# Scalsol/mega.pytorch

Hardware: AMD Instinct MI355X
Metric: frames/sec MEGA R-101 inference, 1000x600 VID clip (higher is better)
Workload: dtype bf16

## Files before the change

### include/mega_hip.h

```cpp
#ifndef MEGA_HIP_H
#define MEGA_HIP_H

#include <stddef.h>

#ifdef __cplusplus
extern "C" {
#endif

#define MEGA_F32 0
#define MEGA_BF16 1
#define MEGA_F16 2

#define MEGA_OK 0
#define MEGA_ERR_ARG 1
#define MEGA_ERR_LAUNCH 2
#define MEGA_ERR_WS 3
#define MEGA_ERR_LIMIT 4

int mega_conv2d_nhwc(const void* in, const void* w, const float* scale, const float* bias, const void* residual,
                     void* out, int N, int H, int W, int Cin, int Cout, int R, int S, int stride, int pad, int dil,
                     int relu, int ldo, int ldr, int in_dtype, int out_dtype, void* stream);
int mega_conv2d_nhwc_tile(int M, int Cout, int K);
int mega_conv2d_nhwc_plan(int M, int Cout, int K, int in_dtype);
int mega_conv2d_nhwc_plan_ex(int N, int H, int W, int Cin, int Cout, int R, int S, int stride, int pad, int dil, int ldo,
                             int has_residual, int in_dtype, int out_dtype);

size_t mega_conv2d_nhwc_workspace_bytes(int M, int Cout, int K);
int mega_conv2d_nhwc_ws(const void* in, const void* w, const float* scale, const float* bias, const void* residual,
                        void* out, int N, int H, int W, int Cin, int Cout, int R, int S, int stride, int pad, int dil,
                        int relu, int ldo, int ldr, int in_dtype, int out_dtype, void* ws, size_t ws_bytes, void* stream);

int mega_conv2d_nhwc_rs(const void* in, const void* w, const float* scale, const float* bias, const void* residual, void* out,
                        int N, int H, int W, int Cin, int Cout, int relu, int ldo, int ldr, int res_H, int res_W, int res_stride,
                        int dtype, void* stream);

int mega_stem_conv_bn_relu(const float* in, const float* w_tap64, const float* scale, const float* bias, void* out,
                           int N, int H, int W, int out_dtype, void* stream);
int mega_stem_conv_bn_relu_bf16(const float* in, const void* w_n176_bf16, const float* scale, const float* bias,
                                void* out, int N, int H, int W, void* stream);
int mega_stem_conv_bn_relu_bf16_u8(const void* frames_u8, const void* w_n176_bf16, const float* scale, const float* bias,
                                   void* out, int N, int H, int W, float mean0, float mean1, float mean2, int to_bgr,
                                   void* stream);

int mega_stem_pool_dt(const void* in, int u8, const void* w_n176, const float* scale, const float* bias, void* out, int N,
                      int H, int W, float mean0, float mean1, float mean2, int to_bgr, int dtype, void* stream);
void mega_stem_pool_tile(int* rows, int* cols);

int mega_maxpool3x3s2_nhwc(const void* in, void* out, int N, int H, int W, int C, int dtype, void* stream);

int mega_avgpool2x2_ceil_nhwc(const void* in, void* out, int N, int H, int W, int C, int dtype, void* stream);

int mega_roi_align_fwd(const void* feat, const float* rois, void* out, int K, int C, int H, int W,
                       float spatial_scale, int pooled_h, int pooled_w, int sampling_ratio, int in_nhwc,
                       int out_nhwc, int dtype, int out_dtype, void* stream);

size_t mega_nms_full_workspace_bytes(int n);
int mega_nms(const float* dets, const float* scores, int n, float thr, int strict_gt, long long* keep_out,
             int* keep_cnt, void* ws, size_t ws_bytes, void* stream);

size_t mega_nms_workspace_bytes(int P, int nmax);
int mega_nms_sorted(const float* boxes, const int* counts, const unsigned char* valid, const int* order, int P,
                    int nmax, float thr, int strict_gt, int max_keep, int* keep_pos, int* keep_cnt,
                    unsigned char* flags, void* ws, size_t ws_bytes, void* stream);

size_t mega_rpn_select_workspace_bytes(int B, int pre_nms_top_n);
int mega_rpn_select_idx(const float* rpn_out, const float* cell_anchors, int B, int Hf, int Wf, int A, int ldc,
                        int anchor_stride, int pre_nms_top_n, int post_nms_top_n, float nms_thresh, int strict_gt,
                        float min_size, float im_w, float im_h, float* proposals, float* prop_scores, int* prop_cnt,
                        int* prop_index, void* ws, size_t ws_bytes, void* stream);

size_t mega_postprocess_workspace_bytes(int R, int NC);
int mega_postprocess(const float* logits, const float* deltas, const float* props, const int* nprop, int R, int NC,
                     float wx, float wy, float ww, float wh, float im_w, float im_h, float score_thresh,
                     float nms_thresh, int strict_gt, int max_det, float* out_boxes, float* out_scores,
                     long long* out_labels, int* out_cnt, float* probs_out, void* ws, size_t ws_bytes,
                     void* stream);

size_t mega_postprocess_batched_workspace_bytes(int B, int R, int NC);
int mega_postprocess_batched(const float* logits, const float* deltas, const float* props, const int* nprop, int B,
                             int R, int NC, float wx, float wy, float ww, float wh, float im_w, float im_h,
                             float score_thresh, float nms_thresh, int strict_gt, int max_det, float* out_boxes,
                             float* out_scores, long long* out_labels, int* out_cnt, float* probs_out, void* ws,
                             size_t ws_bytes, void* stream);

int mega_postprocess_candidates_batched(const float* logits, const float* deltas, const float* props, const int* nprop,
                                        int B, int R, int NC, float wx, float wy, float ww, float wh, float im_w,
                                        float im_h, float score_thresh, float* cboxes, float* cscores, void* stream);

size_t mega_bbox_aug_merge_workspace_bytes(int F, int K, int R, int NC);
int mega_bbox_aug_merge(const float* cboxes, const float* cscores, int F, int K, int R, int NC, const int* view_w,
                        const int* view_h, const int* view_flip, float score_thresh, float nms_thresh, int strict_gt,
                        int max_det, float* out_boxes, float* out_scores, long long* out_labels, int* out_cnt, void* ws,
                        size_t ws_bytes, void* stream);

size_t mega_soft_merge_workspace_bytes(int F, int K, int R, int NC);
int mega_soft_merge(const float* cboxes, const float* cscores, int F, int K, int R, int NC, const int* view_w,
                    const int* view_h, const int* view_flip, float score_thresh, float nms_thresh, int strict_gt,
                    int soft_method, float sigma, int vote, float vote_thresh, int vote_scoring, int max_det,
                    float* out_boxes, float* out_scores, long long* out_labels, int* out_cnt, void* ws, size_t ws_bytes,
                    void* stream);

int mega_position_logits(const float* rois_q, const float* rois_k, const float* wg_t, const float* bg,
                         const float* dim_mat, float* out, int Nq, int Nk, int ldp, int precise, void* stream);

int mega_relation_attention(const void* q, int ldq, const void* k, int ldk, const void* vt, int ldv,
                            const float* pos, int ldp, const void* resid, int ldr, const float* bias_v, void* out,
                            int ldo, int Nq, int Nk, int groups, float scale, int dtype, void* ws, size_t ws_bytes,
                            void* stream);
int mega_relation_attention_splits(int Nq, int Nk, int groups);
size_t mega_relation_attention_workspace_bytes(int Nq, int Nk, int groups);

int mega_preprocess_frames(const unsigned char* in, float* out, int N, int H, int W, float mean0, float mean1,
                           float mean2, int to_bgr, void* stream);

int mega_resize_bilinear_u8(const unsigned char* in, unsigned char* out, unsigned char* tmp, int N, int Hi, int Wi,
                            int Ho, int Wo, const int* bounds_h, const int* coef_h, int ksize_h, const int* bounds_v,
                            const int* coef_v, int ksize_v, void* stream);
int mega_resize_bilinear_u8_flip(const unsigned char* in, unsigned char* out, unsigned char* tmp, int N, int Hi, int Wi,
                                 int Ho, int Wo, const int* bounds_h, const int* coef_h, int ksize_h,
                                 const int* bounds_v, const int* coef_v, int ksize_v, int hflip, void* stream);

int mega_fgfa_warp_aggregate(const void* feats, const float* flow, void* out, float* weights_out, int T, int H,
                             int W, int Cf, int Ce, int key, int dtype, void* stream);
int mega_fgfa_warp_aggregate_ring(const void* feats, const float* flow, void* out, float* weights_out, int T, int H,
                                  int W, int Cf, int Ce, const int* order, int dtype, void* stream);

int mega_fgfa_pair_taps(const float* ring, long long ring_stride, const float* cur, long long cur_stride, const int* order,
                        void* out, int T, int H, int W, int dtype, void* stream);

int mega_dff_warp_scale(const void* feats, const float* flow, const void* scale, void* out, int H, int W, int C,
                        int dtype, void* stream);

int mega_copy_segments(const void* segs, int n, void* stream);

int mega_bottleneck64_fwd_dt(const void* x, const void* w1, const float* s1, const float* b1, const void* w2, const float* s2,
                             const float* b2, const void* w3, const float* s3, const float* b3, void* out, int N, int H, int W,
                             int dtype, void* stream);

int mega_bottleneck64_even_fwd_dt(const void* x, const void* w1, const float* s1, const float* b1, const void* w2, const float* s2,
                                  const float* b2, const void* w3, const float* s3, const float* b3, void* out, int N, int H, int W,
                                  int dtype, void* stream);

int mega_bottleneck64_ds_fwd_dt(const void* x, const void* w1, const float* s1, const float* b1, const void* w2, const float* s2,
                                const float* b2, const void* w3, const float* s3, const float* b3, const void* wd, const float* sd,
                                const float* bd, void* out, int N, int H, int W, int dtype, void* stream);

int mega_split_f32_to_bf16x3(const float* src, void* dst_bf16, int rows, int K, void* stream);


int mega_split_f32_to_planes_dt(const float* src, void* dst, int rows, int K, int dtype, void* stream);

int mega_roi_align_fwd_planes_dt(const float* feat, const float* rois, void* out_planes, int K, int C, int H, int W,
                                 float spatial_scale, int pooled_h, int pooled_w, int sampling_ratio, int dtype, void* stream);

int mega_conv2d_nhwc_sp_dt(const void* in, int ldi, int kwrap, const void* w, const float* scale, const float* bias,
                           const void* residual, int ldr, void* out, int ldo, int out_mode, int N, int H, int W, int Cin,
                           int Cout, int R, int S, int stride, int pad, int dil, int relu, int dtype, void* ws, size_t ws_bytes,
                           void* stream);


int mega_copy_cast_segments_dt(const void* segs, int n, int dtype, void* stream);

int mega_cast_f32_to_half(const float* src, void* dst, size_t n, int dtype, void* stream);

const char* mega_last_error_string(void);

typedef struct {
  const void* q; const void* k; const void* vt; const float* pos; const void* pos_tiled; const void* resid;
  const float* bias_v; void* out; void* ws; size_t ws_bytes;
  int ldq, ldk, ldv, ldp, ldr, ldo, Nq, Nk;
  int io_f32;
  int nk1;
  const void* k2;
  const void* vt2;
  int ldv2;
  int reserved;
} mega_attn_desc;
int mega_relation_attention_batched(const void* descs , int n, int groups,
                                    float scale, int dtype, void* stream);

typedef struct { const float* rois_q; const float* rois_k; void* out_bf16; int Nq, Nk; } mega_pos_desc;

int mega_position_logits_tiled_dt(const float* rois_q, const float* rois_k, const float* wg_t, const float* bg,
                                  const float* dim_mat, void* out16, int Nq, int Nk, int dtype, void* stream);
int mega_position_logits_tiled_batched_dt(const void* descs , int n, const float* wg_t,
                                          const float* bg, const float* dim_mat, int dtype, void* stream);
int mega_relation_attention_tiled_pos_dt(const void* q, int ldq, const void* k, int ldk, const void* vt, int ldv,
// ... 75 lines not shown
```

### mega/pytorch_amd/_lib.py

```python
import ctypes
import os

HERE = os.path.dirname(os.path.abspath(__file__))
LIB_PATH = os.path.join(HERE, "libmega_hip.so")

c_int, c_float, c_void_p, c_size_t = ctypes.c_int, ctypes.c_float, ctypes.c_void_p, ctypes.c_size_t
c_longlong = ctypes.c_longlong

_ERR = {1: "bad argument", 2: "kernel launch failure", 3: "workspace too small", 4: "kernel loop bound exceeded"}

SIGNATURES = {
    "mega_conv2d_nhwc": (c_int, [c_void_p] * 6 + [c_int] * 15 + [c_void_p]),
    "mega_conv2d_nhwc_ws": (c_int, [c_void_p] * 6 + [c_int] * 15 + [c_void_p, c_size_t, c_void_p]),
    "mega_conv2d_nhwc_workspace_bytes": (c_size_t, [c_int] * 3),
    "mega_conv2d_nhwc_rs": (c_int, [c_void_p] * 6 + [c_int] * 12 + [c_void_p]),
    "mega_stem_conv_bn_relu": (c_int, [c_void_p] * 5 + [c_int] * 4 + [c_void_p]),
    "mega_stem_conv_bn_relu_bf16": (c_int, [c_void_p] * 5 + [c_int] * 3 + [c_void_p]),
    "mega_stem_conv_bn_relu_bf16_u8": (c_int, [c_void_p] * 5 + [c_int] * 3 + [c_float] * 3 + [c_int, c_void_p]),
    "mega_stem_pool_dt": (c_int, [c_void_p, c_int] + [c_void_p] * 4 + [c_int] * 3 + [c_float] * 3 + [c_int, c_int, c_void_p]),
    "mega_stem_pool_tile": (None, [c_void_p, c_void_p]),
    "mega_maxpool3x3s2_nhwc": (c_int, [c_void_p] * 2 + [c_int] * 5 + [c_void_p]),
    "mega_avgpool2x2_ceil_nhwc": (c_int, [c_void_p] * 2 + [c_int] * 5 + [c_void_p]),
    "mega_roi_align_fwd": (c_int, [c_void_p] * 3 + [c_int] * 4 + [c_float] + [c_int] * 7 + [c_void_p]),
    "mega_nms_full_workspace_bytes": (c_size_t, [c_int]),
    "mega_nms": (c_int, [c_void_p, c_void_p, c_int, c_float, c_int, c_void_p, c_void_p, c_void_p, c_size_t, c_void_p]),
    "mega_nms_workspace_bytes": (c_size_t, [c_int, c_int]),
    "mega_nms_sorted": (c_int, [c_void_p] * 4 + [c_int, c_int, c_float, c_int, c_int] + [c_void_p] * 4 +
                        [c_size_t, c_void_p]),
    "mega_rpn_select_workspace_bytes": (c_size_t, [c_int, c_int]),
    "mega_rpn_select_idx": (c_int, [c_void_p, c_void_p] + [c_int] * 8 + [c_float, c_int, c_float, c_float, c_float] +
                            [c_void_p] * 5 + [c_size_t, c_void_p]),
    "mega_postprocess_workspace_bytes": (c_size_t, [c_int, c_int]),
    "mega_postprocess": (c_int, [c_void_p] * 4 + [c_int, c_int] + [c_float] * 8 + [c_int, c_int] + [c_void_p] * 6 +
                         [c_size_t, c_void_p]),
    "mega_postprocess_batched_workspace_bytes": (c_size_t, [c_int, c_int, c_int]),
    "mega_postprocess_batched": (c_int, [c_void_p] * 4 + [c_int, c_int, c_int] + [c_float] * 8 + [c_int, c_int] +
                                 [c_void_p] * 6 + [c_size_t, c_void_p]),
    "mega_postprocess_candidates_batched": (c_int, [c_void_p] * 4 + [c_int] * 3 + [c_float] * 7 + [c_void_p] * 3),
    "mega_bbox_aug_merge_workspace_bytes": (c_size_t, [c_int] * 4),
    "mega_bbox_aug_merge": (c_int, [c_void_p, c_void_p] + [c_int] * 4 + [c_void_p] * 3 + [c_float, c_float, c_int, c_int] +
                            [c_void_p] * 5 + [c_size_t, c_void_p]),
    "mega_soft_merge_workspace_bytes": (c_size_t, [c_int] * 4),
    "mega_soft_merge": (c_int, [c_void_p, c_void_p] + [c_int] * 4 + [c_void_p] * 3 +
                        [c_float, c_float, c_int, c_int, c_float, c_int, c_float, c_int, c_int] + [c_void_p] * 5 +
                        [c_size_t, c_void_p]),
    "mega_position_logits": (c_int, [c_void_p] * 6 + [c_int] * 4 + [c_void_p]),
    "mega_relation_attention_splits": (c_int, [c_int, c_int, c_int]),
    "mega_relation_attention_workspace_bytes": (c_size_t, [c_int, c_int, c_int]),
    "mega_relation_attention": (c_int, [c_void_p, c_int, c_void_p, c_int, c_void_p, c_int, c_void_p, c_int,
                                        c_void_p, c_int, c_void_p, c_void_p, c_int, c_int, c_int, c_int, c_float,
                                        c_int, c_void_p, c_size_t, c_void_p]),
    "mega_relation_attention_batched": (c_int, [c_void_p, c_int, c_int, c_float, c_int, c_void_p]),
    "mega_position_logits_tiled_dt": (c_int, [c_void_p] * 6 + [c_int] * 3 + [c_void_p]),
    "mega_position_logits_tiled_batched_dt": (c_int, [c_void_p, c_int, c_void_p, c_void_p, c_void_p, c_int, c_void_p]),
    "mega_relation_attention_tiled_pos_dt": (c_int, [c_void_p, c_int, c_void_p, c_int, c_void_p, c_int, c_void_p,
                                                     c_void_p, c_int, c_void_p, c_void_p, c_int, c_int, c_int, c_int,
                                                     c_float, c_int, c_void_p, c_size_t, c_void_p]),
    "mega_conv2d_nhwc_tile": (c_int, [c_int] * 3),
    "mega_conv2d_nhwc_plan": (c_int, [c_int] * 4),
    "mega_conv2d_nhwc_plan_ex": (c_int, [c_int] * 14),
    "mega_preprocess_frames": (c_int, [c_void_p, c_void_p] + [c_int] * 3 + [c_float] * 3 + [c_int, c_void_p]),
    "mega_dff_warp_scale": (c_int, [c_void_p] * 4 + [c_int] * 4 + [c_void_p]),
    "mega_fgfa_pair_taps": (c_int, [c_void_p, c_longlong, c_void_p, c_longlong, c_void_p, c_void_p] + [c_int] * 4 + [c_void_p]),
    "mega_resize_bilinear_u8": (c_int, [c_void_p] * 3 + [c_int] * 5 + [c_void_p, c_void_p, c_int, c_void_p, c_void_p,
                                                                      c_int, c_void_p]),
    "mega_resize_bilinear_u8_flip": (c_int, [c_void_p] * 3 + [c_int] * 5 + [c_void_p, c_void_p, c_int, c_void_p,
                                                                           c_void_p, c_int, c_int, c_void_p]),
    "mega_fgfa_warp_aggregate": (c_int, [c_void_p] * 4 + [c_int] * 7 + [c_void_p]),
    "mega_fgfa_warp_aggregate_ring": (c_int, [c_void_p] * 4 + [c_int] * 5 + [c_void_p, c_int, c_void_p]),
    "mega_copy_segments": (c_int, [c_void_p, c_int, c_void_p]),
    "mega_bottleneck64_fwd_dt": (c_int, [c_void_p] * 11 + [c_int] * 4 + [c_void_p]),
    "mega_bottleneck64_even_fwd_dt": (c_int, [c_void_p] * 11 + [c_int] * 4 + [c_void_p]),
    "mega_bottleneck64_ds_fwd_dt": (c_int, [c_void_p] * 14 + [c_int] * 4 + [c_void_p]),
    "mega_cast_f32_to_half": (c_int, [c_void_p, c_void_p, c_size_t, c_int, c_void_p]),
    "mega_copy_cast_segments_dt": (c_int, [c_void_p, c_int, c_int, c_void_p]),
    "mega_split_f32_to_bf16x3": (c_int, [c_void_p, c_void_p, c_int, c_int, c_void_p]),
    "mega_split_f32_to_planes_dt": (c_int, [c_void_p, c_void_p, c_int, c_int, c_int, c_void_p]),
    "mega_roi_align_fwd_planes_dt": (c_int, [c_void_p] * 3 + [c_int] * 4 + [c_float] + [c_int] * 4 + [c_void_p]),
    "mega_conv2d_nhwc_sp_dt": (c_int, [c_void_p, c_int, c_int, c_void_p, c_void_p, c_void_p, c_void_p, c_int, c_void_p, c_int,
                                       c_int] + [c_int] * 12 + [c_void_p, c_size_t, c_void_p]),
    "mega_conv2d_nhwc_ks_workspace_bytes": (c_size_t, [c_int] * 5),
    "mega_conv2d_nhwc_ks": (c_int, [c_void_p] * 6 + [c_int] * 16 + [c_void_p, c_size_t, c_void_p]),
    "mega_conv2d_nhwc_subpixel": (c_int, [c_void_p] * 4 + [c_int] * 13 + [c_void_p, c_size_t, c_void_p]),
    "mega_flow_level_assemble": (c_int, [c_void_p] * 5 + [c_int] * 10 + [c_void_p]),
    "mega_flow_pred_finish": (c_int, [c_void_p, c_int, c_void_p, c_float, c_void_p] + [c_int] * 4 + [c_void_p]),
    "mega_flow_conv1_combine": (c_int, [c_void_p, c_void_p, c_void_p, c_int, c_void_p, c_int, c_longlong, c_int, c_int, c_void_p]),
    "mega_fgfa_warp_aggregate_ring_pos": (c_int, [c_void_p] * 4 + [c_int] * 5 + [c_void_p, c_int, c_int, c_void_p]),
    "mega_fgfa_warp_aggregate_ring_pos_batched": (c_int, [c_void_p] * 4 + [c_int] * 5 + [c_void_p, c_int, c_int, c_int, c_void_p]),
    "mega_vid_eval_match": (c_int, [c_void_p] * 10 + [c_int] * 3 + [c_longlong, c_int] + [c_void_p] * 4),
    "mega_vid_eval_workspace_bytes": (c_size_t, [c_longlong, c_int, c_int]),
    "mega_vid_eval_ap": (c_int, [c_void_p] * 5 + [c_int, c_int, c_longlong] + [c_void_p] * 2 + [c_size_t, c_void_p]),
    "mega_proposal_recall_match": (c_int, [c_void_p] * 7 + [c_int, c_int, c_longlong, c_longlong, c_int, c_int] +
                                   [c_void_p] * 3),
    "mega_seq_nms_workspace_bytes": (c_size_t, [c_longlong, c_longlong]),
    "mega_seq_nms": (c_int, [c_void_p] * 4 + [c_int] * 3 + [c_longlong, c_float, c_float, c_int] + [c_void_p] * 4 +
                     [c_size_t, c_void_p]),
    "mega_link_tracks_workspace_bytes": (c_size_t, [c_int, c_int]),
    "mega_link_tracks": (c_int, [c_void_p] * 5 + [c_int] * 3 + [c_longlong, c_float, c_float, c_int, c_int] +
                         [c_void_p] * 5 + [c_size_t, c_void_p]),
    "mega_tubelet_match_workspace_bytes": (c_size_t, [c_longlong]),
    "mega_tubelet_match": (c_int, [c_void_p] * 14 + [c_int] * 4 + [c_longlong] * 7 + [c_void_p] * 5 + [c_size_t, c_void_p]),
    "mega_tubelet_scores": (c_int, [c_void_p, c_void_p, c_longlong, c_longlong, c_int, c_void_p, c_void_p]),
    "mega_motion_iou_workspace_bytes": (c_size_t, [c_longlong, c_int, c_int]),
    "mega_motion_iou": (c_int, [c_void_p] * 5 + [c_int, c_longlong, c_int, c_int] + [c_void_p] * 3 + [c_size_t, c_void_p]),
    "mega_overlay_detections_workspace_bytes": (c_size_t, [c_int, c_int]),
    "mega_overlay_detections": (c_int, [c_void_p, c_int, c_int, c_int, c_void_p, c_void_p, c_void_p, c_int, c_void_p, c_int,
                                        c_float, c_float, c_float, c_int, c_void_p, c_int, c_void_p, c_int, c_void_p,
                                        c_void_p, c_void_p, c_int, c_int, c_int, c_int, c_void_p, c_size_t, c_void_p]),
    "mega_last_error_string": (ctypes.c_char_p, []),
}

_lib = None


def load():
    global _lib
    if _lib is not None:
        return _lib
    if not os.path.exists(LIB_PATH):
        raise RuntimeError(
            "libmega_hip.so not found at %s -- run `python -c 'import __graft_entry__ as g; g.build()'` "
            "(there is no CPU fallback for the MEGA hot path)" % LIB_PATH)
    import torch
    lib = ctypes.CDLL(LIB_PATH)
    for name, (res, args) in SIGNATURES.items():
        fn = getattr(lib, name)
        fn.restype = res
        fn.argtypes = args
    _lib = lib
    return lib


def check(rc, what):
    if rc != 0:
        detail = ""
        if rc == 2 and _lib is not None:
            detail = ": " + _lib.mega_last_error_string().decode()
        raise RuntimeError("%s failed: %s (code %d)%s" % (what, _ERR.get(rc, "unknown"), rc, detail))
```

### mega/pytorch_amd/build.py

```python
import hashlib
import os
import subprocess
import sys

HERE = os.path.dirname(os.path.abspath(__file__))
CSRC = os.path.join(HERE, "csrc")
LIB = os.path.join(HERE, "libmega_hip.so")
STAMP = os.path.join(HERE, "csrc", ".build_stamp")
SOURCES = {
    "igemm.hip": [],
    "igemm8.hip": [],
    "spatial.hip": [],
    "boxes.hip": ["-ffp-contract=off"],
    "relation.hip": ["-mllvm", "-amdgpu-mfma-vgpr-form=1"],
    "frames.hip": ["-ffp-contract=off"],
    "fgfa.hip": [],
    "assemble.hip": [],
    "conv64.hip": [],
    "bneck64.hip": [],
    "vid_eval.hip": ["-ffp-contract=off"],
    "seq_nms.hip": ["-ffp-contract=off"],
    "tracks.hip": ["-ffp-contract=off"],
    "bbox_aug.hip": ["-ffp-contract=off"],
    "soft_nms.hip": ["-ffp-contract=off"],
    "overlay.hip": ["-ffp-contract=off"],
    "proposal_recall.hip": ["-ffp-contract=off"],
    "track_eval.hip": ["-ffp-contract=off"],
    "motion_iou.hip": ["-ffp-contract=off"],
}
HIPCC = os.environ.get("HIPCC", "/opt/rocm/bin/hipcc")
BASE_FLAGS = ["--offload-arch=gfx950", "-O3", "-std=c++17", "-fPIC", "-Wno-unused-result"]


def _probe_flags(flags):
    if not flags or not os.path.exists(HIPCC):
        return list(flags)
    import tempfile
    with tempfile.TemporaryDirectory() as td:
        src = os.path.join(td, "probe.hip")
        with open(src, "w") as f:
            f.write("#include <hip/hip_runtime.h>\n__global__ void mega_probe() {}\n")
        cmd = [HIPCC, "--offload-arch=gfx950", "-O1"] + list(flags) + ["-c", src, "-o", os.path.join(td, "probe.o")]
        if subprocess.run(cmd, stdout=subprocess.PIPE, stderr=subprocess.STDOUT).returncode == 0:
            return list(flags)
    sys.stderr.write("build.py: hipcc rejects %s -- building without it\n" % " ".join(flags))
    return []


def _digest():
    h = hashlib.sha256()
    for fn in sorted(os.listdir(CSRC)):
        if fn.endswith((".hip", ".h")):
            h.update(fn.encode())
            h.update(open(os.path.join(CSRC, fn), "rb").read())
    h.update(" ".join(BASE_FLAGS).encode())
    h.update(repr(sorted(SOURCES.items())).encode())
    h.update(open(os.path.abspath(__file__), "rb").read())
    return h.hexdigest()


def build(force=False, verbose=False):
    dig = _digest()
    if not force and os.path.exists(LIB) and os.path.exists(STAMP) and open(STAMP).read().strip() == dig:
        return LIB
    if not os.path.exists(HIPCC):
        if os.path.exists(LIB):
            return LIB
        raise RuntimeError("hipcc not found at %s and no prebuilt %s" % (HIPCC, LIB))
    objs = []
    procs = []
    for src, extra in SOURCES.items():
        path = os.path.join(CSRC, src)
        if not os.path.exists(path):
            continue
        if "-mllvm" in extra:
            extra = _probe_flags(extra)
        obj = os.path.join(CSRC, src.replace(".hip", ".o"))
        cmd = [HIPCC] + BASE_FLAGS + extra + ["-c", path, "-o", obj]
        if verbose:
            print(" ".join(cmd))
        procs.append((src, subprocess.Popen(cmd, stdout=subprocess.PIPE, stderr=subprocess.STDOUT)))
        objs.append(obj)
    for src, pr in procs:
        out, _ = pr.communicate()
        if pr.returncode != 0:
            raise RuntimeError("hipcc failed on %s:\n%s" % (src, out.decode()))
        if verbose and out:
            print(out.decode())
    cmd = [HIPCC, "--offload-arch=gfx950", "-shared", "-fPIC", "-o", LIB] + objs
    subprocess.check_call(cmd)
    with open(STAMP, "w") as f:
        f.write(dig)
    return LIB


if __name__ == "__main__":
    print(build(force="--force" in sys.argv, verbose=True))
```

### mega/pytorch_amd/csrc/igemm8.hip

```cpp
#include <type_traits>

#include "launch.h"
#include "igemm_params.h"

namespace {

constexpr int NT8 = 512;
constexpr int ROWB = 128;
constexpr int HALF = 128 * ROWB;
constexpr int LDS8 = 8 * HALF;
constexpr int LDS8_ALLOC = 2 * 64 * (256 + 4) * 4 > LDS8 ? 2 * 64 * (256 + 4) * 4 : LDS8;
__host__ __device__ constexpr int slot_a(int i, int par) { return (i * 2 + par) * HALF; }
__host__ __device__ constexpr int slot_b(int j, int par) { return 4 * HALF + (j * 2 + par) * HALF; }
constexpr unsigned OOB = 0x80000000u;

typedef __attribute__((address_space(3))) void* lds_ptr_t;

struct KPos {
  int kc, ks, kr, dh, dw;
  unsigned uni;
};

constexpr int EPI_PLAIN = 0;
constexpr int EPI_SUBPIXEL = 6;
// ... 425 lines not shown
      if (so) {
        if (res) {
          if (p.relu == 1) run(std::true_type{}, std::true_type{}, std::true_type{}); else run(std::true_type{}, std::false_type{}, std::true_type{});
        } else {
          if (p.relu == 1) run(std::false_type{}, std::true_type{}, std::true_type{}); else run(std::false_type{}, std::false_type{}, std::true_type{});
        }
      }
    }
    if (!so) {
      if (res) {
        if (p.relu == 1) run(std::true_type{}, std::true_type{}, std::false_type{}); else run(std::true_type{}, std::false_type{}, std::false_type{});
      } else {
        if (p.relu == 1) run(std::false_type{}, std::true_type{}, std::false_type{}); else run(std::false_type{}, std::false_type{}, std::false_type{});
      }
    }
    return;
  }
  if (SP && p.ksplit == 1) return;
  if (RS) return;
  const bool res_vec = res != nullptr && vec_ok && sizeof(OT) == 2 && p.ksplit == 1;
  uint4 rres2[2][NIT];
  auto load_res = [&](int i, int f, uint4 (&dst)[NIT]) {
    const int wrows = i == 1 ? WROWS1 : 64;
#pragma unroll
    for (int it = 0; it < NIT; ++it) {
      const int e = tid + it * NT8;
      const int row = e / VPR, cv = e - row * VPR;
      const int m = m0 + i * 128 + (row >> 5) * wrows + f * 32 + (row & 31), n = n0 + cv * OVE;
      dst[it] = make_uint4(0, 0, 0, 0);
      if (m < p.M && n + OVE <= p.Cout) dst[it] = *reinterpret_cast<const uint4*>(res + (size_t)m * p.ldr + n);
    }
  };
  auto scb = [&](int n, float x) {
    const float sc = (p.ksplit == 1 && p.scale && n < p.Cout) ? p.scale[n] : 1.f;
    const float bi = (p.ksplit == 1 && p.bias && n < p.Cout) ? p.bias[n] : 0.f;
    return fmaf(x, sc, bi);
  };
  if (res_vec) {
    load_res(0, 0, rres2[0]);
    load_res(0, 1, rres2[1]);
  }
#pragma unroll
  for (int i = 0; i < 2; ++i) {
#pragma unroll
    for (int f = 0; f < (i == 1 ? MF1 : 2); ++f) {
      const int wrows = i == 1 ? WROWS1 : 64;
      uint4 (&rres)[NIT] = rres2[f];
      if (i + f > 0) { MEGA_WAIT_LDS(); MEGA_BAR(); }
      stage(cs, i, f);
      MEGA_WAIT_LDS();
      MEGA_BAR();
      if (p.ksplit > 1) {
        float* part = p.partial + (size_t)blockIdx.z * p.M * p.Cout;
        for (int e = tid; e < 64 * (BN / 4); e += NT8) {
          const int row = e / (BN / 4), cv = e - row * (BN / 4);
          const int m = m0 + i * 128 + (row >> 5) * wrows + f * 32 + (row & 31), n = n0 + cv * 4;
          if (m >= p.M || n >= p.Cout) continue;
          const float4 v = *reinterpret_cast<const float4*>(cs + row * CST + cv * 4);
          if (n + 4 <= p.Cout && p.Cout % 4 == 0) {
            *reinterpret_cast<float4*>(part + (size_t)m * p.Cout + n) = v;
          } else {
            const float vv[4] = {v.x, v.y, v.z, v.w};
            for (int t = 0; t < 4 && n + t < p.Cout; ++t) part[(size_t)m * p.Cout + n + t] = vv[t];
          }
        }
        continue;
      }
      if constexpr (!SP) {
#pragma unroll
      for (int it = 0; it < NIT; ++it) {
        const int e = tid + it * NT8;
        const int row = e / VPR, cv = e - row * VPR;
        const int m = m0 + i * 128 + (row >> 5) * wrows + f * 32 + (row & 31), n = n0 + cv * OVE;
        if (m >= p.M || n >= p.Cout) continue;
        float v[OVE];
#pragma unroll
        for (int t = 0; t < OVE; t += 4) {
          const float4 q4 = *reinterpret_cast<const float4*>(cs + row * CST + cv * OVE + t);
          v[t] = scb(n + t, q4.x); v[t + 1] = scb(n + t + 1, q4.y); v[t + 2] = scb(n + t + 2, q4.z); v[t + 3] = scb(n + t + 3, q4.w);
        }
        if (vec_ok && n + OVE <= p.Cout) {
          if (res_vec) {
            const HT* re = reinterpret_cast<const HT*>(&rres[it]);
#pragma unroll
            for (int t = 0; t < OVE; ++t) v[t] += Elem<HT>::ld(re + t);
          } else if (res) {
            for (int t = 0; t < OVE; ++t) v[t] += Elem<HT>::ld(res + (size_t)m * p.ldr + n + t);
          }
          uint4 o;
          OT* oe = reinterpret_cast<OT*>(&o);
#pragma unroll
          for (int t = 0; t < OVE; ++t) Elem<OT>::st(oe + t, act(v[t]));
          *reinterpret_cast<uint4*>(out + (size_t)m * p.ldo + n) = o;
        } else {
          for (int t = 0; t < OVE && n + t < p.Cout; ++t) {
            float x = v[t];
            if (res) x += Elem<HT>::ld(res + (size_t)m * p.ldr + n + t);
            Elem<OT>::st(out + (size_t)m * p.ldo + n + t, act(x));
          }
        }
      }
      if (res_vec && i == 0 && f < MF1) load_res(1, f, rres);
      }
    }
  }
#undef MEGA_LDS_RD
#undef MEGA_WAIT_VM
#undef MEGA_WAIT_LDS
#undef MEGA_BAR
#undef MEGA_MMA
#undef MEGA_SB
#undef MEGA_MMA_IF
}

inline void magic_div(int d, unsigned& mg, unsigned& sh) {
  sh = 0;
  while ((1ull << sh) < (unsigned long long)d) ++sh;
  mg = (unsigned)((((1ull << sh) - (unsigned long long)d) << 32) / (unsigned long long)d + 1ull);
}

template <typename OT, int MF1, int CLS, int EPI, int SP, typename HT>
int launch8(const ConvParams& p0, hipStream_t st) {
  constexpr int BM = 128 + 64 * MF1;
  ConvParams p = p0;
  magic_div(p.Ho * p.Wo, p.mg_howo, p.sh_howo);
  magic_div(p.Wo, p.mg_wo, p.sh_wo);
  const int ntm = cdiv(p.M, BM), ntn = cdiv(p.Cout, 256);
  return launch_lds(igemm8_kernel<OT, MF1, CLS, EPI, SP, HT>, dim3(ntm * ntn, 1, p.ksplit), dim3(NT8), LDS8_ALLOC, st, p);
}

bool admit_sp(const ConvParams& p, int out_f32) {
  const size_t oplanes = p.split_out ? 2 : 1, osz = out_f32 ? 4 : 2;
  return p.ldi >= (p.kwrap > 0 ? p.kwrap : p.Cin) && p.ldi % 64 == 0 && (p.kwrap == 0 || (p.kwrap % 64 == 0 && p.kwrap < p.Cin && p.Cin - p.kwrap <= p.kwrap)) &&
         p.Cout % 8 == 0 && !(p.split_out && out_f32) && p.ldo % (out_f32 ? 4 : 8) == 0 && p.ldo >= (int)oplanes * p.Cout &&
         (!p.res || (p.ldr % 8 == 0 && p.ldr >= 2 * p.Cout)) &&
         ((size_t)(p.M - 1) * p.ldo + oplanes * p.Cout) * osz < 0x7FF00000ull &&
         (!p.res || ((size_t)(p.M - 1) * p.ldr + 2 * (size_t)p.Cout) * 2 < 0x7FF00000ull) &&
         (p.ksplit == 1 || (!p.split_out && !p.res));
}
bool admit_subpixel(const ConvParams& p, int out_f32) {
  return !(p.sp || out_f32 || p.res || p.ksplit != 1 || p.Cout % 256 != 0 || p.ps_C % 8 != 0 || p.ldo % 8 != 0 || p.ps_coff % 8 != 0 ||
           (size_t)p.N * p.ps_H * p.ps_W * p.ldo * 2 >= 0x7FF00000ull);
}
bool admit_strided_res(const ConvParams& p, int out_f32) {
  return !(p.sp || out_f32 || p.ksplit != 1 || !mega_igemm8_streaming(p.R * p.S, p.K) || p.stride != 1 || p.pad != 0 ||
           p.Cout % 256 != 0 || p.ldo % 8 != 0 || p.ldr % 8 != 0 || p.ldr < p.Cout ||
           (long)(p.Ho - 1) * p.rs_stride >= p.rs_H || (long)(p.Wo - 1) * p.rs_stride >= p.rs_W ||
           ((size_t)(p.M - 1) * p.ldo + p.Cout) * 2 >= 0x7FF00000ull ||
           (((size_t)p.N * p.rs_H * p.rs_W - 1) * p.ldr + p.Cout) * 2 >= 0x7FF00000ull);
}

template <typename HT, int EPI, int SP>
int launch8_mode(const ConvParams& p, int bm, int out_f32, hipStream_t st) {
  auto rows = [&](auto ot, auto cls) -> int {
    using OT = decltype(ot);
    constexpr int CLS = decltype(cls)::value;
    if (bm == 256) return launch8<OT, 2, CLS, EPI, SP, HT>(p, st);
    if (bm == 192) return launch8<OT, 1, CLS, EPI, SP, HT>(p, st);
    return MEGA_ERR_ARG;
  };
  using C0 = std::integral_constant<int, 0>;
  using C1 = std::integral_constant<int, 1>;
  if constexpr (EPI == EPI_SUBPIXEL) {
    return rows(HT{}, C0{});
  } else if constexpr (EPI == EPI_STRIDED_RES) {
    return rows(HT{}, C1{});
  } else {
    if (mega_igemm8_streaming(p.R * p.S, p.K) && p.ksplit == 1) return out_f32 ? rows(float{}, C1{}) : rows(HT{}, C1{});
    return out_f32 ? rows(float{}, C0{}) : rows(HT{}, C0{});
  }
}

}

int mega_igemm8_streaming(int taps, int K) { return taps == 1 && K <= 512; }

int mega_igemm8_supports(const ConvParams& p) {
  return p.Cin % 64 == 0 && p.in_bytes < 0x7FF00000u && p.w_bytes < 0x7FF00000u && (p.K >> 6) >= 1;
}

int mega_igemm8_launch(const ConvParams& p, int bm, int out_f32, int half_dtype, hipStream_t st) {
  return dispatch_half(half_dtype, [&](auto tag) -> int {
    using HT = decltype(tag);
    if (p.ps) return admit_subpixel(p, out_f32) ? launch8_mode<HT, EPI_SUBPIXEL, 0>(p, bm, out_f32, st) : MEGA_ERR_ARG;
    if (conv_res_strided(p)) return admit_strided_res(p, out_f32) ? launch8_mode<HT, EPI_STRIDED_RES, 0>(p, bm, out_f32, st) : MEGA_ERR_ARG;
    if (p.sp) return admit_sp(p, out_f32) ? launch8_mode<HT, EPI_PLAIN, 1>(p, bm, out_f32, st) : MEGA_ERR_ARG;
    return launch8_mode<HT, EPI_PLAIN, 0>(p, bm, out_f32, st);
  });
}
```

### mega/pytorch_amd/csrc/igemm_params.h

```cpp
#pragma once
#include <hip/hip_runtime.h>

struct ConvParams {
  const void* in;
  const void* w;
  const float* scale;
  const float* bias;
  const void* res;
  void* out;
  int N, H, W, Cin, Cout, R, S, stride, pad, dil, Ho, Wo;
  int M, K;
  int ldo, ldr;
  int relu;
  unsigned in_bytes, w_bytes;
  int ksplit;
  float* partial;
  int sp;
  int ldi;
  int kwrap;
  int split_out;
  unsigned mg_howo, sh_howo, mg_wo, sh_wo;
  int ps;
  union { int ps_H, rs_H; };
  union { int ps_W, rs_W; };
  union { int ps_C, rs_stride; };
  int ps_crop, ps_coff;
};

inline bool conv_res_strided(const ConvParams& p) { return !p.ps && p.res && p.rs_stride > 1; }

int mega_igemm8_launch(const ConvParams& p, int bm, int out_f32, int half_dtype, hipStream_t st);
int mega_igemm8_supports(const ConvParams& p);
int mega_igemm8_streaming(int taps, int K);
int mega_conv64_supports(const ConvParams& p, int out_f32);
int mega_conv64_launch(const ConvParams& p, int half_dtype, hipStream_t st);
```

Measured before the change: 956.6.

## Add persistent two-blocks-per-CU 1x1 conv kernel with phase-staggered start

Adds a new persistent 1x1 convolution GEMM kernel (128x256 tiles, 256 threads, K-step 32, three-stage LDS ring via buffer_load_lds) sized so two blocks fit per CU. It is routed in for streaming 1x1 convs with K<=256 and enough tiles. Half the blocks sleep for a computed phase delay so the two co-resident blocks alternate between memory and compute phases. The aim is better overlap of loads and MFMA than the existing 512-thread kernel for small-K bottleneck 1x1 layers. The cost is an extra code path and a heuristic delay that may leave the CU idle.

```diff
diff --git a/include/mega_hip.h b/include/mega_hip.h
--- a/include/mega_hip.h
+++ b/include/mega_hip.h
@@ -33,6 +33,10 @@
 int mega_conv2d_nhwc_rs(const void* in, const void* w, const float* scale, const float* bias, const void* residual, void* out,
                         int N, int H, int W, int Cin, int Cout, int relu, int ldo, int ldr, int res_H, int res_W, int res_stride,
                         int dtype, void* stream);
+
+int mega_conv1x1_two_tiles(const void* in, const void* w, const float* scale, const float* bias, const void* residual, void* out,
+                           int N, int H, int W, int Cin, int Cout, int relu, int ldo, int ldr, int res_H, int res_W,
+                           int res_stride, int dtype, int out_f32, int phase_delay, void* stream);
 
 int mega_stem_conv_bn_relu(const float* in, const float* w_tap64, const float* scale, const float* bias, void* out,
                            int N, int H, int W, int out_dtype, void* stream);
diff --git a/mega/pytorch_amd/_lib.py b/mega/pytorch_amd/_lib.py
--- a/mega/pytorch_amd/_lib.py
+++ b/mega/pytorch_amd/_lib.py
@@ -14,6 +14,7 @@
     "mega_conv2d_nhwc_ws": (c_int, [c_void_p] * 6 + [c_int] * 15 + [c_void_p, c_size_t, c_void_p]),
     "mega_conv2d_nhwc_workspace_bytes": (c_size_t, [c_int] * 3),
     "mega_conv2d_nhwc_rs": (c_int, [c_void_p] * 6 + [c_int] * 12 + [c_void_p]),
+    "mega_conv1x1_two_tiles": (c_int, [c_void_p] * 6 + [c_int] * 14 + [c_void_p]),
     "mega_stem_conv_bn_relu": (c_int, [c_void_p] * 5 + [c_int] * 4 + [c_void_p]),
     "mega_stem_conv_bn_relu_bf16": (c_int, [c_void_p] * 5 + [c_int] * 3 + [c_void_p]),
     "mega_stem_conv_bn_relu_bf16_u8": (c_int, [c_void_p] * 5 + [c_int] * 3 + [c_float] * 3 + [c_int, c_void_p]),
diff --git a/mega/pytorch_amd/build.py b/mega/pytorch_amd/build.py
--- a/mega/pytorch_amd/build.py
+++ b/mega/pytorch_amd/build.py
@@ -10,6 +10,7 @@
 SOURCES = {
     "igemm.hip": [],
     "igemm8.hip": [],
+    "igemm8s.hip": [],
     "spatial.hip": [],
     "boxes.hip": ["-ffp-contract=off"],
     "relation.hip": ["-mllvm", "-amdgpu-mfma-vgpr-form=1"],
diff --git a/mega/pytorch_amd/csrc/igemm8.hip b/mega/pytorch_amd/csrc/igemm8.hip
--- a/mega/pytorch_amd/csrc/igemm8.hip
+++ b/mega/pytorch_amd/csrc/igemm8.hip
@@ -601,6 +601,10 @@
 
 template <typename HT, int EPI, int SP>
 int launch8_mode(const ConvParams& p, int bm, int out_f32, hipStream_t st) {
+  if constexpr (SP == 0 && (EPI == EPI_PLAIN || EPI == EPI_STRIDED_RES)) {
+    if (mega_igemm8_streaming(p.R * p.S, p.K) && p.ksplit == 1 && mega_igemm8s_admits(p, out_f32) && mega_igemm8s_wants(p))
+      return mega_igemm8s_launch(p, out_f32, Half16<HT>::CODE, -1, st);
+  }
   auto rows = [&](auto ot, auto cls) -> int {
     using OT = decltype(ot);
     constexpr int CLS = decltype(cls)::value;
diff --git a/mega/pytorch_amd/csrc/igemm8s.hip b/mega/pytorch_amd/csrc/igemm8s.hip
--- /dev/null
+++ b/mega/pytorch_amd/csrc/igemm8s.hip
@@ -0,0 +1,373 @@
+#include <type_traits>
+
+#include "launch.h"
+#include "igemm_params.h"
+
+namespace {
+
+constexpr int NTS = 256;
+constexpr int KTS = 32;
+constexpr int ROWBS = KTS * 2;
+constexpr int ASTG = 128 * ROWBS;
+constexpr int BSTG = 256 * ROWBS;
+constexpr int BBASE = 3 * ASTG;
+constexpr int RINGS = 3 * (ASTG + BSTG);
+constexpr int CSTS = 256 + 4;
+constexpr int LDSS_ALLOC = 64 * CSTS * 4 > RINGS ? 64 * CSTS * 4 : RINGS;
+static_assert(LDSS_ALLOC <= 80 * 1024, "two blocks per CU");
+constexpr unsigned OOBS = 0x80000000u;
+constexpr int EPIS_PLAIN = 0, EPIS_STRIDED_RES = 7;
+constexpr int MAX_DELAY = 256;
+
+typedef __attribute__((address_space(3))) void* ldss_ptr_t;
+
+__device__ __forceinline__ int fast_divs(int n, unsigned mg, unsigned sh) {
+  return (int)((__umulhi((unsigned)n, mg) + (unsigned)n) >> sh);
+}
+
+template <typename OT, int EPI, typename HT>
+__global__ __launch_bounds__(NTS, 2) void igemm8s_kernel(ConvParams p) {
+  static_assert(sizeof(OT) == 4 || std::is_same<OT, HT>::value, "16-bit outputs have the operands' type");
+  constexpr int BM = 128, BN = 256;
+  constexpr bool RS = EPI == EPIS_STRIDED_RES;
+  constexpr bool CAN_RES = sizeof(OT) == 2;
+  extern __shared__ __attribute__((aligned(16))) unsigned char smem[];
+
+  const int tid = threadIdx.x;
+  const int lane = tid & 63;
+  const int wave = __builtin_amdgcn_readfirstlane(tid >> 6);
+  const int wr = wave >> 1, wc = wave & 1;
+
+  const __amdgpu_buffer_rsrc_t rs_in = __builtin_amdgcn_make_buffer_rsrc(const_cast<void*>(p.in), 0, (int)p.in_bytes, 0x00020000);
+  const __amdgpu_buffer_rsrc_t rs_w = __builtin_amdgcn_make_buffer_rsrc(const_cast<void*>(p.w), 0, (int)p.w_bytes, 0x00020000);
+  const bool has_res = CAN_RES && p.res != nullptr;
+  const __amdgpu_buffer_rsrc_t rs_res = __builtin_amdgcn_make_buffer_rsrc(
+      const_cast<void*>(has_res ? p.res : p.out), 0,
+      has_res ? (int)(((size_t)(RS ? p.N * p.rs_H * p.rs_W - 1 : p.M - 1) * p.ldr + (size_t)p.Cout) * 2) : 0, 0x00020000);
+  const __amdgpu_buffer_rsrc_t rs_out = __builtin_amdgcn_make_buffer_rsrc(
+      p.out, 0, (int)(((size_t)(p.M - 1) * p.ldo + p.Cout) * sizeof(OT)), 0x00020000);
+
+  const int prow = tid >> 2, pch = tid & 3;
+  const unsigned lcb = (unsigned)((pch ^ ((prow >> 2) & 3)) * 16);
+  unsigned char* const wbase = smem + wave * 1024;
+
+  const int l31 = lane & 31;
+  unsigned a_rd[2], b_rd[2];
+#pragma unroll
+  for (int ks = 0; ks < 2; ++ks) {
+    const unsigned ch = (unsigned)(((ks * 2 + (lane >> 5)) ^ ((l31 >> 2) & 3)) * 16);
+    a_rd[ks] = (unsigned)((wr * 64 + l31) * ROWBS) + ch;
+    b_rd[ks] = (unsigned)(BBASE + (wc * 128 + l31) * ROWBS) + ch;
+  }
+
+#define MS_RD(dst, addr, imm) asm volatile("ds_read_b128 %0, %1 offset:%2" : "=v"(dst) : "v"(addr), "n"(imm) : "memory")
+#define MS_WAIT_VM(n) asm volatile("s_waitcnt vmcnt(%0)" ::"n"(n) : "memory")
+#define MS_WAIT_LGKM(n)                                  \
+  do {                                                   \
+    asm volatile("s_waitcnt lgkmcnt(%0)" ::"n"(n) : "memory"); \
+    __builtin_amdgcn_sched_barrier(0);                   \
+  } while (0)
+#define MS_BAR()                      \
+  do {                                \
+    asm volatile("" ::: "memory");   \
+    __builtin_amdgcn_s_barrier();     \
+    asm volatile("" ::: "memory");   \
+  } while (0)
+#define MS_SB() __builtin_amdgcn_sched_barrier(0)
+
+  constexpr int OVE = 16 / (int)sizeof(OT);
+  constexpr int VPR = BN / OVE;
+  constexpr int NIT = 64 * VPR / NTS;
+  constexpr int RSTEP = NTS / VPR;
+  const int row0 = tid / VPR, cv0 = (tid % VPR) * OVE;
+  const float neg_slope = p.relu == 1 ? 0.f : (p.relu == 2 ? 0.1f : 1.f);
+  auto act = [&](float x) { return x > 0.f ? x : x * neg_slope; };
+  float* const cs = reinterpret_cast<float*>(smem);
+  const bool al16 = ((reinterpret_cast<size_t>(p.scale) | reinterpret_cast<size_t>(p.bias)) & 15) == 0;
+
+  const int nkt = p.K / KTS;
+  const int ntn = (p.Cout + BN - 1) / BN;
+  const int ntiles = ((p.M + BM - 1) / BM) * ntn;
+  const int HoWo = p.Ho * p.Wo;
+  int delay = (int)blockIdx.x * 2 >= (int)gridDim.x ? min(max(p.phase_delay, 0), MAX_DELAY) : 0;
+
+  for (int vt = blockIdx.x; vt < ntiles; vt += gridDim.x) {
+    int lid;
+    {
+      const int q = ntiles >> 3, r = ntiles & 7, xcd = vt & 7, loc = vt >> 3;
+      lid = (xcd < r ? xcd * (q + 1) : r * (q + 1) + (xcd - r) * q) + loc;
+    }
+    const int tile_m = lid / ntn, tile_n = lid - tile_m * ntn;
+    const int m0 = tile_m * BM, n0 = tile_n * BN;
+    const int ncol = n0 + cv0;
+
+    unsigned a_off[2];
+#pragma unroll
+    for (int u = 0; u < 2; ++u) {
+      const int m = m0 + u * 64 + prow;
+      const bool ok = m < p.M;
+      const int mm = ok ? m : 0;
+      const int nimg = fast_divs(mm, p.mg_howo, p.sh_howo);
+      const int rem = mm - nimg * HoWo;
+      const int ho = fast_divs(rem, p.mg_wo, p.sh_wo);
+      const int wo = rem - ho * p.Wo;
+      const int hi = ho * p.stride - p.pad, wi = wo * p.stride - p.pad;
+      const bool in = ok & ((unsigned)hi < (unsigned)p.H) & ((unsigned)wi < (unsigned)p.W);
+      a_off[u] = in ? ((unsigned)(nimg * p.H * p.W) + (unsigned)(hi * p.W + wi)) * (unsigned)(p.Cin * 2) + lcb : OOBS;
+    }
+    unsigned b_off[4];
+#pragma unroll
+    for (int u = 0; u < 4; ++u) {
+      const int n = n0 + u * 64 + prow;
+      b_off[u] = n < p.Cout ? (unsigned)n * (unsigned)(p.K * 2) + lcb : OOBS;
+    }
+    int tnext = 0;
+    auto issue_tile = [&](int sa, int sb) {
+      const unsigned dead = tnext < nkt ? 0u : OOBS;
+      const unsigned kb = (unsigned)(tnext * ROWBS);
+#pragma unroll
+      for (int u = 0; u < 2; ++u)
+        __builtin_amdgcn_raw_ptr_buffer_load_lds(rs_in, (ldss_ptr_t)(wbase + sa + u * 4096), 16, (a_off[u] + kb) | dead, 0, 0, 0);
+#pragma unroll
+      for (int u = 0; u < 4; ++u)
+        __builtin_amdgcn_raw_ptr_buffer_load_lds(rs_w, (ldss_ptr_t)(wbase + BBASE + sb + u * 4096), 16, (b_off[u] + kb) | dead, 0, 0, 0);
+      ++tnext;
+    };
+
+    auto slab_m = [&](int f, int it) { return (m0 + row0) + (((it * RSTEP) >> 5) * 64 + f * 32 + ((it * RSTEP) & 31)); };
+    auto res_off = [&](int f, int it) -> unsigned {
+      const int m = slab_m(f, it);
+      if constexpr (RS) {
+        const int t = fast_divs(m, p.mg_howo, p.sh_howo), rem = m - t * HoWo;
+        const int y = fast_divs(rem, p.mg_wo, p.sh_wo), x = rem - y * p.Wo;
+        return m < p.M ? (unsigned)(((t * p.rs_H + y * p.rs_stride) * p.rs_W + x * p.rs_stride) * p.ldr + ncol) * 2u : OOBS;
+      } else {
+        return (unsigned)(m * p.ldr + ncol) * 2u;
+      }
+    };
+
+    u32x4_t rr[2][CAN_RES ? NIT : 1];
+    if constexpr (CAN_RES) {
+#pragma unroll
+      for (int it = 0; it < NIT; ++it) rr[0][it] = __builtin_amdgcn_raw_buffer_load_b128(rs_res, res_off(0, it), 0, 0);
+    }
+
+    issue_tile(0, 0);
+    issue_tile(ASTG, BSTG);
+
+    for (; delay > 0; --delay) __builtin_amdgcn_s_sleep(8);
+
+    f32x16_t acc[2][4];
+#pragma unroll
+    for (int f = 0; f < 2; ++f)
+#pragma unroll
+      for (int j = 0; j < 4; ++j)
+#pragma unroll
+        for (int r = 0; r < 16; ++r) acc[f][j][r] = 0.f;
+
+    u32x4_t af[2][2], bfr[2][4];
+    int sa = 0, sb = 0;
+    int na = 2 * ASTG, nb = 2 * BSTG;
+    for (int t = 0; t < nkt; ++t) {
+      MS_WAIT_VM(6);
+      MS_WAIT_LGKM(0);
+      MS_BAR();
+      issue_tile(na, nb);
+      const unsigned aa0 = a_rd[0] + (unsigned)sa, aa1 = a_rd[1] + (unsigned)sa;
+      const unsigned ba0 = b_rd[0] + (unsigned)sb, ba1 = b_rd[1] + (unsigned)sb;
+      MS_RD(af[0][0], aa0, 0); MS_RD(af[0][1], aa0, 2048);
+      MS_RD(bfr[0][0], ba0, 0); MS_RD(bfr[0][1], ba0, 2048); MS_RD(bfr[0][2], ba0, 4096); MS_RD(bfr[0][3], ba0, 6144);
+      MS_RD(af[1][0], aa1, 0); MS_RD(af[1][1], aa1, 2048);
+      MS_RD(bfr[1][0], ba1, 0); MS_RD(bfr[1][1], ba1, 2048); MS_RD(bfr[1][2], ba1, 4096); MS_RD(bfr[1][3], ba1, 6144);
+      MS_WAIT_LGKM(6);
+#pragma unroll
+      for (int f = 0; f < 2; ++f)
+#pragma unroll
+        for (int j = 0; j < 4; ++j) acc[f][j] = Half16<HT>::mfma32(bfr[0][j], af[0][f], acc[f][j]);
+      MS_SB();
+      MS_WAIT_LGKM(0);
+#pragma unroll
+      for (int f = 0; f < 2; ++f)
+#pragma unroll
+        for (int j = 0; j < 4; ++j) acc[f][j] = Half16<HT>::mfma32(bfr[1][j], af[1][f], acc[f][j]);
+      MS_SB();
+      sa = sa == 2 * ASTG ? 0 : sa + ASTG;
+      sb = sb == 2 * BSTG ? 0 : sb + BSTG;
+      na = na == 2 * ASTG ? 0 : na + ASTG;
+      nb = nb == 2 * BSTG ? 0 : nb + BSTG;
+    }
+    MS_WAIT_VM(0);
+    MS_BAR();
+
+    float scv[OVE], biv[OVE];
+#pragma unroll
+    for (int t = 0; t < OVE; t += 4) {
+      f32x4_t s4 = {1.f, 1.f, 1.f, 1.f}, b4 = {0.f, 0.f, 0.f, 0.f};
+      if (al16) {
+        if (p.scale) s4 = *reinterpret_cast<const f32x4_t*>(p.scale + ncol + t);
+        if (p.bias) b4 = *reinterpret_cast<const f32x4_t*>(p.bias + ncol + t);
+      } else {
+#pragma unroll
+        for (int u = 0; u < 4; ++u) {
+          if (p.scale) s4[u] = p.scale[ncol + t + u];
+          if (p.bias) b4[u] = p.bias[ncol + t + u];
+        }
+      }
+#pragma unroll
+      for (int u = 0; u < 4; ++u) { scv[t + u] = s4[u]; biv[t + u] = b4[u]; }
+    }
+    if constexpr (CAN_RES) {
+#pragma unroll
+      for (int it = 0; it < NIT; ++it) rr[1][it] = __builtin_amdgcn_raw_buffer_load_b128(rs_res, res_off(1, it), 0, 0);
+    }
+    auto stage = [&](int f) {
+      float* dst = cs + (wr * 32 + l31) * CSTS + wc * 128 + 4 * (lane >> 5);
+#pragma unroll
+      for (int j = 0; j < 4; ++j)
+#pragma unroll
+        for (int g = 0; g < 4; ++g) {
+          const f32x4_t q = {acc[f][j][4 * g], acc[f][j][4 * g + 1], acc[f][j][4 * g + 2], acc[f][j][4 * g + 3]};
+          *reinterpret_cast<f32x4_t*>(dst + j * 32 + 8 * g) = q;
+        }
+    };
+    auto run = [&](auto HR, auto RL) {
+      constexpr bool HAS_RES = decltype(HR)::value;
+      constexpr bool RELU = decltype(RL)::value;
+#pragma unroll
+      for (int f = 0; f < 2; ++f) {
+        if (f > 0) { MS_WAIT_LGKM(0); MS_BAR(); }
+        stage(f);
+        MS_WAIT_LGKM(0);
+        MS_BAR();
+#pragma unroll
+        for (int it = 0; it < NIT; ++it) {
+          const int row = row0 + it * RSTEP;
+          float v[OVE];
+#pragma unroll
+          for (int t = 0; t < OVE; t += 4) {
+            const float4 q4 = *reinterpret_cast<const float4*>(cs + row * CSTS + cv0 + t);
+            v[t] = fmaf(q4.x, scv[t], biv[t]); v[t + 1] = fmaf(q4.y, scv[t + 1], biv[t + 1]);
+            v[t + 2] = fmaf(q4.z, scv[t + 2], biv[t + 2]); v[t + 3] = fmaf(q4.w, scv[t + 3], biv[t + 3]);
+          }
+          if constexpr (HAS_RES) {
+            u32x4_t r4 = rr[f][it];
+            asm volatile("" : "+v"(r4));
+#pragma unroll
+            for (int d = 0; d < 4; ++d) {
+              v[2 * d] += Half16<HT>::lo(r4[d]);
+              v[2 * d + 1] += Half16<HT>::hi(r4[d]);
+            }
+          }
+          const unsigned ooff = (unsigned)(slab_m(f, it) * p.ldo + ncol) * (unsigned)sizeof(OT);
+          u32x4_t o;
+          if constexpr (sizeof(OT) == 2) {
+#pragma unroll
+            for (int d = 0; d < 4; ++d) {
+              if constexpr (RELU) {
+                const s16x2_t z = {0, 0};
+                o[d] = __builtin_bit_cast(unsigned, __builtin_elementwise_max(__builtin_bit_cast(s16x2_t, Half16<HT>::pack2(v[2 * d], v[2 * d + 1])), z));
+              } else {
+                o[d] = Half16<HT>::pack2(act(v[2 * d]), act(v[2 * d + 1]));
+              }
+            }
+          } else {
+#pragma unroll
+            for (int t = 0; t < 4; ++t) o[t] = __float_as_uint(RELU ? fmaxf(v[t], 0.f) : act(v[t]));
+          }
+          __builtin_amdgcn_raw_buffer_store_b128(o, rs_out, ooff, 0, 0);
+        }
+      }
+    };
+    if (has_res) {
+      if constexpr (CAN_RES) {
+        if (p.relu == 1) run(std::true_type{}, std::true_type{}); else run(std::true_type{}, std::false_type{});
+      }
+    } else {
+      if (p.relu == 1) run(std::false_type{}, std::true_type{}); else run(std::false_type{}, std::false_type{});
+    }
+    MS_WAIT_LGKM(0);
+    MS_BAR();
+  }
+#undef MS_RD
+#undef MS_WAIT_VM
+#undef MS_WAIT_LGKM
+#undef MS_BAR
+#undef MS_SB
+}
+
+inline void magic_divs(int d, unsigned& mg, unsigned& sh) {
+  sh = 0;
+  while ((1ull << sh) < (unsigned long long)d) ++sh;
+  mg = (unsigned)((((1ull << sh) - (unsigned long long)d) << 32) / (unsigned long long)d + 1ull);
+}
+
+inline int tiles_of(const ConvParams& p) { return cdiv(p.M, 128) * cdiv(p.Cout, 256); }
+
+inline int default_delay(const ConvParams& p, int out_f32, int grid) {
+  if (tiles_of(p) < 4 * grid) return 0;
+  const long bytes = 128L * p.K * 2 + 128L * 256 * (out_f32 ? 4 : 2) + (p.res ? 128L * 256 * 2 : 0);
+  const long cyc = bytes / 9 > 16L * p.K ? bytes / 9 : 16L * p.K;
+  const long d = cyc / 2 / 512;
+  return (int)(d > MAX_DELAY ? MAX_DELAY : d);
+}
+
+template <typename OT, int EPI, typename HT>
+int launch8s(const ConvParams& p0, int delay, hipStream_t st) {
+  ConvParams p = p0;
+  magic_divs(p.Ho * p.Wo, p.mg_howo, p.sh_howo);
+  magic_divs(p.Wo, p.mg_wo, p.sh_wo);
+  const int ntiles = tiles_of(p), cap = 2 * mega_cu_count(), grid = ntiles < cap ? ntiles : cap;
+  p.phase_delay = delay < 0 ? default_delay(p, sizeof(OT) == 4, grid) : (delay > MAX_DELAY ? MAX_DELAY : delay);
+  return launch_lds(igemm8s_kernel<OT, EPI, HT>, dim3(grid), dim3(NTS), LDSS_ALLOC, st, p);
+}
+
+}
+
+int mega_igemm8s_admits(const ConvParams& p, int out_f32) {
+  if (p.sp || p.ps || p.ksplit != 1 || p.R != 1 || p.S != 1 || p.K != p.Cin) return 0;
+  if (p.Cin % KTS != 0 || p.K < KTS || p.K > 512 || p.in_bytes >= 0x7FF00000u || p.w_bytes >= 0x7FF00000u) return 0;
+  const size_t osz = out_f32 ? 4 : 2;
+  if (p.M <= 0 || p.Cout % 256 != 0 || p.ldo % (int)(16 / osz) != 0 || p.ldo < p.Cout) return 0;
+  if (((size_t)(p.M - 1) * p.ldo + p.Cout) * osz >= 0x7FF00000ull) return 0;
+  if (p.res) {
+    if (out_f32 || p.ldr % 8 != 0 || p.ldr < p.Cout) return 0;
+    const size_t rrows = conv_res_strided(p) ? (size_t)p.N * p.rs_H * p.rs_W : (size_t)p.M;
+    if (((rrows - 1) * p.ldr + p.Cout) * 2 >= 0x7FF00000ull) return 0;
+    if (conv_res_strided(p) && (p.stride != 1 || p.pad != 0 || (long)(p.Ho - 1) * p.rs_stride >= p.rs_H || (long)(p.Wo - 1) * p.rs_stride >= p.rs_W)) return 0;
+  }
+  return 1;
+}
+
+int mega_igemm8s_wants(const ConvParams& p) { return p.K <= 256 && tiles_of(p) >= 2 * mega_cu_count(); }
+
+int mega_igemm8s_launch(const ConvParams& p, int out_f32, int half_dtype, int delay, hipStream_t st) {
+  if (!mega_igemm8s_admits(p, out_f32)) return MEGA_ERR_ARG;
+  return dispatch_half(half_dtype, [&](auto tag) -> int {
+    using HT = decltype(tag);
+    if (conv_res_strided(p)) return launch8s<HT, EPIS_STRIDED_RES, HT>(p, delay, st);
+    return out_f32 ? launch8s<float, EPIS_PLAIN, HT>(p, delay, st) : launch8s<HT, EPIS_PLAIN, HT>(p, delay, st);
+  });
+}
+
+extern "C" int mega_conv1x1_two_tiles(const void* in, const void* w, const float* scale, const float* bias, const void* residual,
+                                      void* out, int N, int H, int W, int Cin, int Cout, int relu, int ldo, int ldr, int res_H,
+                                      int res_W, int res_stride, int dtype, int out_f32, int phase_delay, void* stream) {
+  mega_clear_error();
+  if (!in || !w || !out || N <= 0 || H <= 0 || W <= 0 || Cin <= 0 || Cout <= 0 || res_stride < 1) return MEGA_ERR_ARG;
+  if ((size_t)N * H * W >= 0x7FF00000ull || (size_t)N * H * W * Cin * 2 >= 0x7FF00000ull || (size_t)Cout * Cin * 2 >= 0x7FF00000ull) return MEGA_ERR_ARG;
+  ConvParams p = {};
+  p.in = in; p.w = w; p.scale = scale; p.bias = bias; p.res = residual; p.out = out;
+  p.N = N; p.H = H; p.W = W; p.Cin = Cin; p.Cout = Cout; p.R = 1; p.S = 1; p.stride = 1; p.pad = 0; p.dil = 1; p.Ho = H; p.Wo = W;
+  p.M = N * H * W; p.K = Cin;
+  p.ldo = ldo > 0 ? ldo : Cout;
+  p.ldr = ldr > 0 ? ldr : Cout;
+  p.relu = relu;
+  p.in_bytes = (unsigned)((size_t)p.M * Cin * 2);
+  p.w_bytes = (unsigned)((size_t)Cout * Cin * 2);
+  p.ksplit = 1;
+  if (res_stride > 1) {
+    if (!residual || res_H <= 0 || res_W <= 0) return MEGA_ERR_ARG;
+    p.rs_H = res_H; p.rs_W = res_W; p.rs_stride = res_stride;
+  }
+  return mega_igemm8s_launch(p, out_f32, dtype, phase_delay, (hipStream_t)stream);
+}
diff --git a/mega/pytorch_amd/csrc/igemm_params.h b/mega/pytorch_amd/csrc/igemm_params.h
--- a/mega/pytorch_amd/csrc/igemm_params.h
+++ b/mega/pytorch_amd/csrc/igemm_params.h
@@ -25,6 +25,7 @@
   union { int ps_W, rs_W; };
   union { int ps_C, rs_stride; };
   int ps_crop, ps_coff;
+  int phase_delay;
 };
 
 inline bool conv_res_strided(const ConvParams& p) { return !p.ps && p.res && p.rs_stride > 1; }
@@ -32,5 +33,8 @@
 int mega_igemm8_launch(const ConvParams& p, int bm, int out_f32, int half_dtype, hipStream_t st);
 int mega_igemm8_supports(const ConvParams& p);
 int mega_igemm8_streaming(int taps, int K);
+int mega_igemm8s_admits(const ConvParams& p, int out_f32);
+int mega_igemm8s_wants(const ConvParams& p);
+int mega_igemm8s_launch(const ConvParams& p, int out_f32, int half_dtype, int delay, hipStream_t st);
 int mega_conv64_supports(const ConvParams& p, int out_f32);
 int mega_conv64_launch(const ConvParams& p, int half_dtype, hipStream_t st);
```

Result: slower. 946.0 (-1.1%).
